# kai-neumann/OrthoSfM

Measured on AMD Instinct MI355X. Metric: image-pairs matched/sec + BA iterations/sec (N images, M tracks) at 1/2/4/8 GPU, higher is better.
Workload: dtype i8; 1 GPU; 50 orthographic images, 20000 SIFT features/img, exhaustive matching (1225 pairs, low-res gate + two-way + cross-check + lists; SURVEY 8d's unit of work: up to, not including, RANSAC-F -- the pass through RANSAC-F is `with_geometric_verification`); views=50, features_per_view=20000, pairs=1225

## Files before the change

### orthosfm_amd/csrc/match_kernels.hip

```cpp
#include <algorithm>

#include "match_kernels.h"

namespace osfm {


typedef int v4i __attribute__((ext_vector_type(4)));
typedef int v16i __attribute__((ext_vector_type(16)));


__device__ __forceinline__ int max3i(int a, int b, int c)
{
    int r;
    asm("v_max3_i32 %0, %1, %2, %3" : "=v"(r) : "v"(a), "v"(b), "v"(c));
    return r;
}
__device__ __forceinline__ int med3a(int a, int b, int c)
{
    int r;
    asm("v_med3_i32 %0, %1, %2, %3" : "=v"(r) : "v"(a), "v"(b), "v"(c));
    return r;
}

constexpr int kGroupTiles = 8;
constexpr int kPipeGroupTiles = 16;
constexpr int kPipeTileBits = 9;
constexpr int kValNone = -(1 << 28);

template <int V> struct IntC { static constexpr int value = V; };

__device__ __forceinline__ void store_colpart(int32_t *best, int32_t *second, unsigned byte_off, const ColPart &v)
{
    int32_t *const pb = reinterpret_cast<int32_t *>(reinterpret_cast<char *>(best) + byte_off);
    int32_t *const ps = reinterpret_cast<int32_t *>(reinterpret_cast<char *>(second) + byte_off);
#ifdef OSFM_COLPART_PLAIN_STORE
    *pb = v.key_best; *ps = v.key_second;
#else
    __builtin_nontemporal_store(v.key_best, pb);
    __builtin_nontemporal_store(v.key_second, ps);
#endif
}
__device__ __forceinline__ void store_colpart_sbase(int32_t *best, int32_t *second, unsigned byte_off, const ColPart &v)
{
    asm volatile("global_store_dword %0, %1, %2 nt" :: "v"(byte_off), "v"(v.key_best), "s"(best) : "memory");
    asm volatile("global_store_dword %0, %1, %2 nt" :: "v"(byte_off), "v"(v.key_second), "s"(second) : "memory");
}

template <int CH, bool MASKED, bool RAW, bool C0>
__device__ __forceinline__ void
tile_body(const MatchProblem &pd, int rb, int seg, RowPart *__restrict__ rowparts,
    ColPart *__restrict__ colparts, char *smem, const int8_t *__restrict__ zero_tile)
{
    static_assert(!C0 || RAW, "the correction-free form needs the raw row operand");
    constexpr int D = CH * 16;
    constexpr int KS = CH / 2;
    constexpr int RPB = 16 / CH;
    constexpr int TILE_BYTES = kTileCols * D;
    constexpr int CHUNKS = kTileCols * CH;
    constexpr int CPT = CHUNKS / 256;
    constexpr int BBUF_BYTES = 2 * TILE_BYTES > 16384 ? 2 * TILE_BYTES : 16384;
    constexpr int kRawShift = C0 ? kPipeTileBits : 7;
    constexpr int kCurNone = RAW ? -(1 << (30 - kRawShift)) : kKeyNone;
    static_assert(kSegCols / kTileCols <= (1 << 7), "tile index must fit the key");
    constexpr bool PIPE = C0;
    constexpr int NCHUNK = 2 * KS;
    constexpr int RPC = 16 / NCHUNK;
    constexpr int CPC = 16 / KS;

    char *bbuf = smem;
    int *corrbuf = reinterpret_cast<int *>(smem + BBUF_BYTES);
    ColPart *colbuf = reinterpret_cast<ColPart *>(smem + BBUF_BYTES + 2 * 64 * 4);
    int *rsecbuf = reinterpret_cast<int *>(smem + BBUF_BYTES + 2 * 64 * 4 + 8 * 4 * 64 * 8);

    const int n1 = pd.n1, n2 = pd.n2, n2stride = pd.n2stride;
    const int8_t *const Bbase = C0 ? pd.B_raw : pd.B;
    const int32_t *const corrBbase = pd.corrB;
    int32_t *const colbest = reinterpret_cast<int32_t *>(colparts + pd.colpart_off) + (int64_t)rb * pd.n2stride;
    int32_t *const colsecond = colbest + (int64_t)pd.nrb * pd.n2stride;
    const int tid = threadIdx.x;
    const int wave = tid >> 6, lane = tid & 63, lr = lane & 31, lh = lane >> 5;
    const int row0 = rb * kRowsPerBlock + wave * 64;
    const int gcode = wave * 2 + lh;

    const int8_t *Abase = pd.A;
    const int32_t *corrA = pd.corrA;
    int arow0 = row0;
    if (RAW) { Abase = pd.A_raw; corrA = pd.corrA_raw; }
    else if (!MASKED && rb >= pd.nrb_main) {
        Abase = pd.A_special; corrA = pd.corrA_special;
        arow0 = (rb - pd.nrb_main) * kRowsPerBlock + wave * 64;
    }
    v4i a[2][KS];
    v16i ra[2];
#pragma unroll
    for (int rf = 0; rf < 2; ++rf) {
        const int8_t *arow = Abase + (size_t)(arow0 + rf * 32 + lr) * D;
#pragma unroll
        for (int ks = 0; ks < KS; ++ks)
            a[rf][ks] = *reinterpret_cast<const v4i *>(arow + (ks * 2 + lh) * 16);
#pragma unroll
        for (int r = 0; r < 16; ++r)
            ra[rf][r] = C0 ? 0 : corrA[arow0 + rf * 32 + (r & 3) + 8 * (r >> 2) + 4 * lh];
    }
    const v16i zero16 = {0, 0, 0, 0, 0, 0, 0, 0, 0, 0, 0, 0, 0, 0, 0, 0};
    unsigned row_valid_bits = 0xffffffffu;
    if (MASKED) {
        row_valid_bits = 0;
#pragma unroll
        for (int fr = 0; fr < 32; ++fr) {
            const int row = row0 + (fr >> 4) * 32 + (fr & 3) + 8 * ((fr >> 2) & 3) + 4 * lh;
            row_valid_bits |= (row < n1 ? 1u : 0u) << fr;
        }
    }

    v16i rbest[2], rcur[2];
#pragma unroll
    for (int rf = 0; rf < 2; ++rf)
#pragma unroll
        for (int r = 0; r < 16; ++r) {
            rbest[rf][r] = kKeyNone; rcur[rf][r] = kCurNone;
            rsecbuf[(rf * 16 + r) * 256 + tid] = kKeyNone;
        }

    const int seg_cols = pd.seg_cols;
    const int col_begin = seg * seg_cols;
    const int col_lim = min(n2, col_begin + seg_cols);
    const int ntiles = (col_lim - col_begin + kTileCols - 1) / kTileCols;

    typedef __attribute__((address_space(3))) void lds_void;
    typedef const __attribute__((address_space(1))) void glb_void;
    int wave_s = __builtin_amdgcn_readfirstlane(wave);
    if (PIPE) asm volatile("" : "+s"(wave_s));
    unsigned lane4 = (unsigned)lane * 4u;
    if (PIPE) asm volatile("" : "+v"(lane4));
    unsigned lane_off[CPT];
#pragma unroll
    for (int c = 0; c < CPT; ++c) {
        const int q = (c * 4 + wave) * 64 + lane;
        const int col = q / CH;
        const int ch = (q % CH) ^ ((col / RPB) % CH);
        lane_off[c] = (unsigned)(col * D + ch * 16);
    }
    auto dma_wait = [&](bool store_behind = false) {
        if (!PIPE) return;
#ifndef OSFM_TILE_WAIT_ALL
        if (store_behind) { asm volatile("s_waitcnt vmcnt(2)" ::: "memory"); return; }
#endif
        asm volatile("s_waitcnt vmcnt(0)" ::: "memory");
    };
    auto tile_src = [&](int t) {
        const int8_t *src = Bbase + (size_t)(col_begin + t * kTileCols) * D;
        if (PIPE && t >= ntiles) src = zero_tile;
        return src;
    };
    auto stage_tile_at = [&](const int8_t *src, int t, int buf) {
#pragma unroll
        for (int c = 0; c < CPT; ++c) {
            const int q0 = (c * 4 + wave_s) * 64;
            if (PIPE) {
                static_assert(!PIPE || RAW, "the PIPE schedule must not contain compiler-managed m0 users");
                const unsigned lds_at = (unsigned)(uintptr_t)(bbuf + buf * TILE_BYTES + q0 * 16);
                asm volatile("s_mov_b32 m0, %2\n\tglobal_load_lds_dwordx4 %0, %1"
                             :: "v"(lane_off[c]), "s"(src), "s"(lds_at) : "memory");
            } else {
                __builtin_amdgcn_global_load_lds(
                    (glb_void *)(src + lane_off[c]),
                    (lds_void *)(uintptr_t)(bbuf + buf * TILE_BYTES + q0 * 16), 16, 0, 0);
            }
        }
        if (!RAW && wave_s == 0)
            __builtin_amdgcn_global_load_lds(
                (glb_void *)(corrBbase + col_begin + t * kTileCols + lane),
                (lds_void *)(uintptr_t)(corrbuf + buf * 64), 4, 0, 0);
    };
    auto stage_tile = [&](int t, int buf) { stage_tile_at(tile_src(t), t, buf); };
    const int8_t *pf_src = nullptr;

    v4i b[2][KS];
    int cb_next[2] = {0, 0};
    auto load_b = [&](int buf, int cf) {
        const int col = cf * 32 + lr;
        const int swz = (col / RPB) % CH;
#pragma unroll
        for (int ks = 0; ks < KS; ++ks)
            b[cf][ks] = *reinterpret_cast<const v4i *>(
                bbuf + buf * TILE_BYTES + col * D + (((ks * 2 + lh) ^ swz) * 16));
        if (!RAW) cb_next[cf] = corrbuf[buf * 64 + col];
    };

    int cbj[2] = {0, 0}, cjt[2] = {0, 0};
    bool col_valid[2] = {true, true};
    int g[2] = {kValNone, kValNone};

    v16i acc0[2], acc1[2];

    auto phase = [&](auto ph_c, auto cl_c, auto mg_c, auto rs_c, auto pre_c, v16i (&cur)[2], v16i (&nxt)[2], int buf_next,
                     int tile0, int tm, int tms) {
        constexpr int PH = decltype(ph_c)::value;
        constexpr bool PRE = decltype(pre_c)::value != 0;
        constexpr int CL = decltype(cl_c)::value;
        constexpr int RS = decltype(rs_c)::value;
        constexpr bool MG = decltype(mg_c)::value != 0;
        constexpr int OF = PH ^ 1;
        int sv = 0;
        ColPart cpm[4];
        if (CL >= 0) sv = rsecbuf[(OF * 16 + CL) * 256 + tid];
        if (MG) {
#pragma unroll
            for (int w = 0; w < 4; ++w) cpm[w] = colbuf[((tm & 7) * 4 + w) * 64 + lane];
        }
#pragma unroll
        for (int i = 0; i < NCHUNK; ++i) {
            const int cf = i / KS, ks = i % KS;
            if (PRE && i == 0)
                ;
            else if (ks == 0)
                nxt[cf] = __builtin_amdgcn_mfma_i32_32x32x32_i8(a[PH ^ 1][0], b[cf][0], C0 ? zero16 : ra[PH ^ 1], 0, 0, 0);
            else
                nxt[cf] = __builtin_amdgcn_mfma_i32_32x32x32_i8(a[PH ^ 1][ks], b[cf][ks], nxt[cf], 0, 0, 0);
            if (PH == 0 && i == KS - 1) load_b(buf_next, 0);
            if (PH == 1 && i == 0) {
                __builtin_amdgcn_sched_barrier(0);
                load_b(buf_next, 1);
            }

#pragma unroll
            for (int r = i * RPC; r < (i + 1) * RPC; ++r) {
                if (RAW) {
                    if (RS >= 0 && r == RS) rcur[PH][r] = max(cur[0][r], cur[1][r]);
                    else rcur[PH][r] = max(max(rcur[PH][r], cur[0][r]), cur[1][r]);
                } else {
                    int k0 = (int)(((unsigned)cur[0][r] << 8) + (unsigned)cjt[0]);
                    int k1 = (int)(((unsigned)cur[1][r] << 8) + (unsigned)cjt[1]);
                    if (MASKED) {
                        k0 = col_valid[0] ? k0 : kKeyNone;
                        k1 = col_valid[1] ? k1 : kKeyNone;
                    }
                    rcur[PH][r] = max3i(rcur[PH][r], k0, k1);
                }
            }
            {
                int x[CPC];
#pragma unroll
                for (int j = 0; j < CPC; ++j) {
                    x[j] = cur[cf][ks * CPC + j];
                    if (MASKED) x[j] = ((row_valid_bits >> (PH * 16 + ks * CPC + j)) & 1u) ? x[j] : kValNone;
                }
                int gg;
                if (PH == 0 && ks == 0) gg = max(x[0], x[1]);
                else gg = max(max(g[cf], x[0]), x[1]);
#pragma unroll
                for (int j = 2; j < CPC; j += 2) gg = max(max(gg, x[j]), x[j + 1]);
                asm volatile("" : "+v"(gg));
                g[cf] = gg;
            }
            if (CL >= 0 && i == 2) {
                const int r = CL;
                const int gk = (int)(((unsigned)rcur[OF][r] << kRawShift) | (unsigned)tile0);
                rsecbuf[(OF * 16 + r) * 256 + tid] = med3a(rbest[OF][r], sv, gk);
                int nb = max(rbest[OF][r], gk);
                if (PIPE) asm volatile("" : "+v"(nb));
                rbest[OF][r] = nb;
            }
            if (MG && (i == 2 || i == 3)) {
                if (i == 2) {
                    int k1 = cpm[0].key_best, k2 = cpm[0].key_second;
#pragma unroll
                    for (int w = 1; w < 4; ++w) {
                        k2 = max(max(min(k1, cpm[w].key_best), k2), cpm[w].key_second);
                        k1 = max(k1, cpm[w].key_best);
                    }
                    cpm[0].key_best = k1; cpm[0].key_second = k2;
                } else {
                    store_colpart_sbase(colbest + col_begin + tms * kTileCols, colsecond + col_begin + tms * kTileCols, lane4, cpm[0]);
                }
            }
            __builtin_amdgcn_sched_barrier(0);
        }
    };

    auto first_mfma = [&]() {
        acc1[0] = __builtin_amdgcn_mfma_i32_32x32x32_i8(a[1][0], b[0][0], C0 ? zero16 : ra[1], 0, 0, 0);
        __builtin_amdgcn_sched_barrier(0);
    };

    stage_tile(0, 0);
    stage_tile(PIPE || ntiles > 1 ? 1 : 0, 1);
    dma_wait();
    __syncthreads();
    load_b(0, 0);
    load_b(0, 1);
#pragma unroll
    for (int cf = 0; cf < 2; ++cf) {
        acc0[cf] = __builtin_amdgcn_mfma_i32_32x32x32_i8(a[0][0], b[cf][0], C0 ? zero16 : ra[0], 0, 0, 0);
#pragma unroll
        for (int ks = 1; ks < KS; ++ks)
            acc0[cf] = __builtin_amdgcn_mfma_i32_32x32x32_i8(a[0][ks], b[cf][ks], acc0[cf], 0, 0, 0);
    }
    if (PIPE) {
        first_mfma();
        pf_src = tile_src(2);
        asm volatile("" : "+s"(pf_src));
    }
    __syncthreads();

    auto tile_top = [&](int t) {
        if (PIPE) {
            stage_tile_at(pf_src, t + 2, t & 1);
            pf_src = tile_src(t + 3);
            asm volatile("" : "+s"(pf_src));
        } else {
            stage_tile(min(t + 2, ntiles - 1), t & 1);
        }
#pragma unroll
        for (int cf = 0; cf < 2; ++cf) {
            if (!RAW) {
                cbj[cf] = cb_next[cf];
                cjt[cf] = (int)(((unsigned)cbj[cf] << 8) + (unsigned)(t * 2 + cf));
                asm volatile("" : "+v"(cjt[cf]));
            }
            col_valid[cf] = (col_begin + t * kTileCols + cf * 32 + lr) < n2;
        }
    };
    auto tile_bottom = [&](int t, bool store_behind = false, bool pre_issue = false) {
        int kk[2];
#pragma unroll
        for (int cf = 0; cf < 2; ++cf) {
            kk[cf] = (int)((unsigned)(g[cf] + cbj[cf]) << 8) | gcode;
            if (MASKED) kk[cf] = g[cf] < -(1 << 27) ? kKeyNone : kk[cf];
        }
        const auto sw = __builtin_amdgcn_permlane32_swap((unsigned)kk[0], (unsigned)kk[1], false, false);
        const int x0 = (int)sw[0], x1 = (int)sw[1];
        ColPart cp;
        cp.key_best = max(x0, x1);
        cp.key_second = min(x0, x1);
        colbuf[((t & 7) * 4 + wave) * 64 + lane] = cp;
        if (pre_issue) first_mfma();
        dma_wait(store_behind);
        __syncthreads();
    };
    auto close_all = [&](auto first_tile) {
        int sv[2][16];
#pragma unroll
        for (int rf = 0; rf < 2; ++rf)
#pragma unroll
            for (int r = 0; r < 16; ++r) sv[rf][r] = rsecbuf[(rf * 16 + r) * 256 + tid];
#pragma unroll
        for (int rf = 0; rf < 2; ++rf)
#pragma unroll
            for (int r = 0; r < 16; ++r) {
                const int gk = RAW ? (int)(((unsigned)rcur[rf][r] << kRawShift) | (unsigned)first_tile(rf, r)) : rcur[rf][r];
                rsecbuf[(rf * 16 + r) * 256 + tid] = med3a(rbest[rf][r], sv[rf][r], gk);
                rbest[rf][r] = max(rbest[rf][r], gk);
                rcur[rf][r] = kCurNone;
            }
    };
    auto merge_tile = [&](int tm) {
        ColPart cp[4];
#pragma unroll
        for (int w = 0; w < 4; ++w) cp[w] = colbuf[((tm & 7) * 4 + w) * 64 + lane];
        int k1 = cp[0].key_best, k2 = cp[0].key_second;
#pragma unroll
        for (int w = 1; w < 4; ++w) {
            k2 = max(max(min(k1, cp[w].key_best), k2), cp[w].key_second);
            k1 = max(k1, cp[w].key_best);
        }
        const int col = col_begin + tm * kTileCols + lane;
        if (col < n2stride) {
            ColPart out;
            out.key_best = k1;
            out.key_second = k2;
            store_colpart(colbest, colsecond, (unsigned)col * 4u, out);
        }
    };

    int t = 0;
    if (PIPE) {
        static_assert(kPipeGroupTiles == 16, "the staggered schedule closes one of 16 slots per phase");
        auto cycle_tile = [&](auto u_c, int t0) {
            constexpr int u = decltype(u_c)::value;
            const int tt = t0 + u;
            tile_top(tt);
            const int bn = (tt & 1) ^ 1;
            const int tm0 = u >= 5 ? tt - 5 : max(tt - 5, 0);
            const int tm = tm0 + wave;
            phase(IntC<0>(), IntC<u>(), IntC<(u & 3) == 1 ? 1 : 0>(), IntC<(u + 15) & 15>(), IntC<1>(), acc0, acc1, bn,
                max(tt - 16, 0), tm, tm0 + wave_s);
            phase(IntC<1>(), IntC<u>(), IntC<0>(), IntC<u>(), IntC<0>(), acc1, acc0, bn, max(tt - 15, 0), 0, 0);
            tile_bottom(tt, (u & 3) == 1, true);
            return tt + 1 >= ntiles;
        };
        for (; t + 16 < ntiles; t += 16) {
            cycle_tile(IntC<0>(), t); cycle_tile(IntC<1>(), t); cycle_tile(IntC<2>(), t); cycle_tile(IntC<3>(), t);
            cycle_tile(IntC<4>(), t); cycle_tile(IntC<5>(), t); cycle_tile(IntC<6>(), t); cycle_tile(IntC<7>(), t);
            cycle_tile(IntC<8>(), t); cycle_tile(IntC<9>(), t); cycle_tile(IntC<10>(), t); cycle_tile(IntC<11>(), t);
            cycle_tile(IntC<12>(), t); cycle_tile(IntC<13>(), t); cycle_tile(IntC<14>(), t); cycle_tile(IntC<15>(), t);
        }
        do {
            if (cycle_tile(IntC<0>(), t)) break;
            if (cycle_tile(IntC<1>(), t)) break;
            if (cycle_tile(IntC<2>(), t)) break;
            if (cycle_tile(IntC<3>(), t)) break;
            if (cycle_tile(IntC<4>(), t)) break;
            if (cycle_tile(IntC<5>(), t)) break;
            if (cycle_tile(IntC<6>(), t)) break;
            if (cycle_tile(IntC<7>(), t)) break;
            if (cycle_tile(IntC<8>(), t)) break;
            if (cycle_tile(IntC<9>(), t)) break;
            if (cycle_tile(IntC<10>(), t)) break;
            if (cycle_tile(IntC<11>(), t)) break;
            if (cycle_tile(IntC<12>(), t)) break;
            if (cycle_tile(IntC<13>(), t)) break;
            if (cycle_tile(IntC<14>(), t)) break;
            cycle_tile(IntC<15>(), t);
        } while (false);
        const int tl = ntiles - 1, ue = tl & 15, t0 = tl & ~15;
        const int tf = max((tl - 1) & ~3, 0);
        if (tf + wave_s <= tl) merge_tile(tf + wave_s);
        if (tf + 4 + wave_s <= tl) merge_tile(tf + 4 + wave_s);
#pragma unroll
        for (int r = 0; r < 16; ++r) rcur[0][r] = r == ue ? kCurNone : rcur[0][r];
        close_all([&](int rf, int r) {
            if (rf) return r <= ue ? t0 + r : max(t0 - 16 + r, 0);
            return r < ue ? t0 + r + 1 : r > ue ? max(t0 - 15 + r, 0) : 0;
        });
        t = ntiles;
        dma_wait();
    }
    const int t_tail = t;
    if (!PIPE)
    for (; t < ntiles; ++t) {
        tile_top(t);
        phase(IntC<0>(), IntC<-1>(), IntC<0>(), IntC<-1>(), IntC<0>(), acc0, acc1, (t & 1) ^ 1, 0, 0, 0);
        phase(IntC<1>(), IntC<-1>(), IntC<0>(), IntC<-1>(), IntC<0>(), acc1, acc0, (t & 1) ^ 1, 0, 0, 0);
        if (PIPE ? t == ntiles - 1 : ((t % kGroupTiles) == kGroupTiles - 1 || t == ntiles - 1)) {
            const int first = PIPE ? t_tail : (t / kGroupTiles) * kGroupTiles;
            close_all([&](int, int) { return first; });
        }
        tile_bottom(t);
        if ((t & 3) == 3 || t == ntiles - 1) {
            const int tm = (t & ~3) + wave;
            if (tm <= t) merge_tile(tm);
        }
    }

    RowPart *rp = rowparts + pd.rowpart_off + (int64_t)seg * ((int64_t)pd.nrb * kRowsPerBlock);
    int *bb = reinterpret_cast<int *>(smem);
    static_assert(BBUF_BYTES + 2 * 64 * 4 + 8 * 4 * 64 * 8 >= 32 * 256 * 4, "the best keys of both fragments must fit in front of rsecbuf");
    __syncthreads();
#pragma unroll
    for (int rf = 0; rf < 2; ++rf)
#pragma unroll
        for (int r = 0; r < 16; ++r) bb[(rf * 16 + r) * 256 + tid] = rbest[rf][r];
    __syncthreads();
    {
        constexpr int SH = RAW ? kRawShift : 8;
        const int r = lane & 15, h = (lane >> 4) & 1, rf = lane >> 5;
        const int base = (rf * 16 + r) * 256 + wave * 64 + h * 32;
        v4i kb[8], ks[8];
#pragma unroll
        for (int j = 0; j < 8; ++j) {
            const int jj = (j + r) & 7;
            kb[j] = *reinterpret_cast<const v4i *>(bb + base + jj * 4);
            ks[j] = *reinterpret_cast<const v4i *>(rsecbuf + base + jj * 4);
        }
        int b1 = kKeyNone, b2 = kKeyNone, smax = kKeyNone;
#pragma unroll
        for (int j = 0; j < 8; ++j)
#pragma unroll
            for (int e = 0; e < 4; ++e) {
                b2 = med3a(b1, b2, kb[j][e]);
                b1 = max(b1, kb[j][e]);
            }
#pragma unroll
        for (int j = 0; j < 8; j += 2)
#pragma unroll
            for (int e = 0; e < 4; ++e) smax = max3i(smax, ks[j][e], ks[j + 1][e]);
        unsigned hit = 0;
#pragma unroll
        for (int j = 7; j >= 0; --j)
#pragma unroll
            for (int e = 3; e >= 0; --e) hit = (hit << 1) | (kb[j][e] == b1 ? 1u : 0u);
        const unsigned rot = __builtin_amdgcn_alignbit(hit, hit, (32 - 4 * r) & 31);
        const int bl = 31 - __builtin_clz(rot | 1u);
        const int sk = max(b2, smax);
        const int row = row0 + rf * 32 + (r & 3) + 8 * (r >> 2) + 4 * h;
        RowPart out;
        out.ip_best = b1 == kKeyNone ? INT_MIN : (b1 >> SH);
        out.ip_second = sk == kKeyNone ? INT_MIN : (sk >> SH);
        out.idx_best = b1 == kKeyNone ? 0
                     : RAW ? col_begin + (b1 & ((1 << kRawShift) - 1)) * kTileCols + bl
                           : col_begin + (b1 & 255) * 32 + bl;
        out.pad = RAW ? 1 : 0;
        rp[row] = out;
    }
}

template <int CH, bool MASKED, bool RAW, bool C0>
__global__ __launch_bounds__(256, 2) void
match_tile_kernel(const MatchProblem *__restrict__ problems, int num_problems, int total_blocks,
    RowPart *__restrict__ rowparts, ColPart *__restrict__ colparts, unsigned long long *__restrict__ clock_probe,
    const int8_t *__restrict__ zero_tile)
{
    extern __shared__ __attribute__((aligned(16))) char smem[];
    const int lin = xcd_remap(blockIdx.x, total_blocks);
    int lo = 0, hi = num_problems - 1;
    while (lo < hi) {
        const int mid = (lo + hi + 1) >> 1;
        if (problems[mid].block_start <= lin) lo = mid; else hi = mid - 1;
    }
    const MatchProblem &pd = problems[lo];
    const int local = lin - pd.block_start;
    const int rb = local / pd.nseg;
    const int seg = local - rb * pd.nseg;
    if (!MASKED && (rb < pd.nrb_main) != RAW) return;
    if (RAW && (pd.c0 != 0) != C0) return;
    if (C0 && clock_probe != nullptr && (blockIdx.x & 1023) == 0) {
        const unsigned long long c0 = (unsigned long long)clock64(), w0 = (unsigned long long)wall_clock64();
        tile_body<CH, MASKED, RAW, C0>(pd, rb, seg, rowparts, colparts, smem, zero_tile);
        const unsigned long long c1 = (unsigned long long)clock64(), w1 = (unsigned long long)wall_clock64();
        if (threadIdx.x == 0) { atomicAdd(clock_probe, c1 - c0); atomicAdd(clock_probe + 1, w1 - w0); }
        return;
    }
    tile_body<CH, MASKED, RAW, C0>(pd, rb, seg, rowparts, colparts, smem, zero_tile);
}

void launch_match_tiles(int ch, bool masked, bool any_special, bool any_c0, bool any_corrected,
    const MatchProblem *d_problems, int num_problems, int total_blocks, RowPart *rowparts,
    ColPart *colparts, hipStream_t s, unsigned long long *clock_probe, const int8_t *zero_tile)
{
    if (total_blocks <= 0) return;
    const int d = ch * 16;
    const size_t lds = std::max<size_t>(2 * (size_t)kTileCols * d, 16384) + 2 * 64 * 4 + 8 * 4 * 64 * sizeof(ColPart) + 32 * 256 * 4;
    const dim3 grid(total_blocks), block(256);
#define OSFM_LAUNCH_TILES(CHV, MASKEDV, RAWV, C0V) \
    for (unsigned long long *PROBE = ((C0V) ? clock_probe : nullptr), *once_ = (unsigned long long *)1; once_; once_ = nullptr) \
    hipLaunchKernelGGL((match_tile_kernel<CHV, MASKEDV, RAWV, C0V>), grid, block, lds, s, d_problems, num_problems, total_blocks, rowparts, colparts, PROBE, zero_tile)
    if (masked) {
        if (ch == 8) OSFM_LAUNCH_TILES(8, true, false, false); else OSFM_LAUNCH_TILES(4, true, false, false);
        return;
    }
    if (any_c0) { if (ch == 8) OSFM_LAUNCH_TILES(8, false, true, true); else OSFM_LAUNCH_TILES(4, false, true, true); }
    if (any_corrected) { if (ch == 8) OSFM_LAUNCH_TILES(8, false, true, false); else OSFM_LAUNCH_TILES(4, false, true, false); }
    if (any_special) { if (ch == 8) OSFM_LAUNCH_TILES(8, false, false, false); else OSFM_LAUNCH_TILES(4, false, false, false); }
#undef OSFM_LAUNCH_TILES
}

__device__ __forceinline__ int match_distance(int ip, const LoweTable &tab)
{
    const int b = max(ip, 0);
    return tab.is_signed ? 32258 - 2 * min(b, 16129) : min(32767, 65025 - min(b, 65025)) * 2;
}

__device__ __forceinline__ int
accept_match(int ip1, int ip2, int idx1, const LoweTable &tab)
{
    const int idx = ip1 >= 0 ? idx1 : 0;
    const int d1 = match_distance(ip1, tab), d2 = match_distance(ip2, tab);
    if (d1 > tab.max_d1) return -1;
    if (d1 >= tab.reject_from[d2 >> 1]) return -1;
    return idx;
}

template <int CTRL, int ROW_MASK = 0xf>
__device__ __forceinline__ int dpp_mov(int v, int old)
{
    return __builtin_amdgcn_update_dpp(old, v, CTRL, ROW_MASK, 0xf, false);
}
constexpr int kDppXor1 = 0xB1;
constexpr int kDppXor2 = 0x4E;
constexpr int kDppHalfMirror = 0x141;
constexpr int kDppMirror = 0x140;
constexpr int kDppBcast15 = 0x142;
constexpr int kDppBcast31 = 0x143;

__device__ __forceinline__ int wave_max(int v)
{
    v = max(v, dpp_mov<kDppXor1>(v, INT_MIN));
    v = max(v, dpp_mov<kDppXor2>(v, INT_MIN));
    v = max(v, dpp_mov<kDppHalfMirror>(v, INT_MIN));
    v = max(v, dpp_mov<kDppMirror>(v, INT_MIN));
    v = max(v, dpp_mov<kDppBcast15, 0xa>(v, INT_MIN));
    v = max(v, dpp_mov<kDppBcast31, 0xc>(v, INT_MIN));
    return __builtin_amdgcn_readlane(v, 63);
}

template <int DIM, int DIR>
__device__ __forceinline__ void
rescan_groups(const MatchProblem &pd, const int (&q)[2], const int (&idx1)[2], const int (&code)[2],
    const int (&kind)[2], int lane, int (&idx_out)[2], int (&best_out)[2], int (&second_out)[2])
{
    constexpr int LPC = DIM / 16;
    constexpr int CPL = 64 / LPC;
    constexpr int NCAND = DIR == 0 ? 2 * kPipeGroupTiles : 32;
    constexpr int J = NCAND / CPL;
    const int c = lane % LPC, k = lane / LPC;
    const int8_t *Q = DIR == 0 ? pd.A : pd.B;
    const int8_t *Cm = DIR == 0 ? pd.B : pd.A;
    const int32_t *corrQ = DIR == 0 ? pd.corrA : pd.corrB;
    const int32_t *corrC = DIR == 0 ? pd.corrB : pd.corrA;

    int cand[2][J], corr_c[2][J], corr_q[2];
    int4 qv[2], cv[2][J];
#pragma unroll
    for (int u = 0; u < 2; ++u) {
        qv[u] = *reinterpret_cast<const int4 *>(Q + (size_t)q[u] * DIM + c * 16);
        corr_q[u] = corrQ[q[u]];
        int base0 = 0, lr = 0, rbase = 0, lh = 0;
        if (DIR == 0) {
            const int seg = idx1[u] / kSegCols, off = idx1[u] - seg * kSegCols;
            lr = off & 31;
            const int tile = off >> 6;
            base0 = seg * kSegCols + (kind[u] ? tile : (tile / kGroupTiles) * kGroupTiles) * kTileCols;
        } else {
            rbase = idx1[u] * kRowsPerBlock + (code[u] >> 1) * 64;
            lh = code[u] & 1;
        }
#pragma unroll
        for (int j = 0; j < J; ++j) {
            const int n = j * CPL + k;
            int cd;
            if (kind[u] >= 3) {
                cd = idx1[u] + (kind[u] == 3 ? 128 : 32) * n;
                if (cd >= (DIR == 0 ? pd.n2 : pd.n1)) cd = -1;
            } else if (DIR == 0) {
                cd = base0 + (n >> 1) * kTileCols + (n & 1) * 32 + lr;
                if (cd >= pd.n2 || (!kind[u] && n >= 2 * kGroupTiles)) cd = -1;
            } else {
                const int r = n & 15;
                cd = rbase + (n >> 4) * 32 + (r & 3) + 8 * (r >> 2) + 4 * lh;
                if (idx1[u] < pd.nrb_main && cd >= pd.n1) cd = -1;
            }
            cand[u][j] = cd;
        }
        if (DIR == 1 && kind[u] < 3 && idx1[u] >= pd.nrb_main) {
#pragma unroll
            for (int j = 0; j < J; ++j) {
                const int sidx = cand[u][j] - pd.nrb_main * kRowsPerBlock;
                cand[u][j] = sidx < pd.n_special ? pd.special_map[sidx] : -1;
            }
        }
    }
#pragma unroll
    for (int u = 0; u < 2; ++u) {
#pragma unroll
        for (int j = 0; j < J; ++j) {
            const int cs = max(cand[u][j], 0);
            cv[u][j] = *reinterpret_cast<const int4 *>(Cm + (size_t)cs * DIM + c * 16);
            corr_c[u][j] = corrC[cs];
        }
    }
#pragma unroll
    for (int u = 0; u < 2; ++u) {
        int kbest = INT_MIN, ksec = INT_MIN;
#pragma unroll
        for (int j = 0; j < J; ++j) {
            int acc = __builtin_amdgcn_sdot4(qv[u].x, cv[u][j].x, 0, false);
            acc = __builtin_amdgcn_sdot4(qv[u].y, cv[u][j].y, acc, false);
            acc = __builtin_amdgcn_sdot4(qv[u].z, cv[u][j].z, acc, false);
            acc = __builtin_amdgcn_sdot4(qv[u].w, cv[u][j].w, acc, false);
            acc += dpp_mov<kDppXor1>(acc, 0);
            acc += dpp_mov<kDppXor2>(acc, 0);
            if (LPC == 8) acc += dpp_mov<kDppHalfMirror>(acc, 0);
            const int key = cand[u][j] >= 0 ? (acc + corr_q[u] + corr_c[u][j]) * 32 + (j * CPL + k) : INT_MIN;
            ksec = med3a(kbest, ksec, key);
            kbest = max(kbest, key);
        }
        const int wbest = wave_max(kbest);
        const int wsec = wave_max(kbest == wbest ? ksec : kbest);
        const int pos = wbest & 31;
        int widx = 0;
#pragma unroll
        for (int j = 0; j < J; ++j)
            if ((pos / CPL) == j) widx = __builtin_amdgcn_readlane(cand[u][j], (pos % CPL) * LPC);
        idx_out[u] = max(widx, 0);
        best_out[u] = wbest >> 5;
        second_out[u] = wsec == INT_MIN ? INT_MIN : wsec >> 5;
    }
}

template <int DIM>
__device__ __forceinline__ void
scan_specials(const MatchProblem &pd, int dir, int q, int lane, int &best_out, int &second_out, int &idx_out)
{
    constexpr int LPC = DIM / 16, CPL = 64 / LPC;
    const int c = lane % LPC, k = lane / LPC;
    const int8_t *Q = dir == 0 ? pd.A : pd.B;
    const int8_t *Cm = dir == 0 ? pd.B_special : pd.A_special;
    const int32_t *corrC = dir == 0 ? pd.corrB_special : pd.corrA_special;
    const int32_t *map = dir == 0 ? pd.special_map_B : pd.special_map;
    const int ns = dir == 0 ? pd.nsB : pd.nsA;
    const int4 qv = *reinterpret_cast<const int4 *>(Q + (size_t)q * DIM + c * 16);
    const int corr_q = (dir == 0 ? pd.corrA : pd.corrB)[q];
    int kbest = INT_MIN, ksec = INT_MIN;
    for (int base = 0; base < ns; base += CPL) {
        const int slot = base + k;
        const bool live = slot < ns;
        const int4 cv = *reinterpret_cast<const int4 *>(Cm + (size_t)(live ? slot : 0) * DIM + c * 16);
        int acc = __builtin_amdgcn_sdot4(qv.x, cv.x, 0, false);
        acc = __builtin_amdgcn_sdot4(qv.y, cv.y, acc, false);
        acc = __builtin_amdgcn_sdot4(qv.z, cv.z, acc, false);
        acc = __builtin_amdgcn_sdot4(qv.w, cv.w, acc, false);
        acc += dpp_mov<kDppXor1>(acc, 0);
        acc += dpp_mov<kDppXor2>(acc, 0);
        if (LPC == 8) acc += dpp_mov<kDppHalfMirror>(acc, 0);
        const int key = live ? (acc + corr_q + corrC[live ? slot : 0]) * 512 + slot : INT_MIN;
        ksec = med3a(kbest, ksec, key);
        kbest = max(kbest, key);
    }
    const int wbest = wave_max(kbest);
    const int wsec = wave_max(kbest == wbest ? ksec : kbest);
    best_out = wbest >> 9;
    second_out = wsec == INT_MIN ? INT_MIN : wsec >> 9;
    idx_out = map[wbest & 511];
}

#ifndef OSFM_FINISH_BATCH
#define OSFM_FINISH_BATCH 16
#endif

constexpr int kFinishThreads = 256, kFinishTurns = 4, kFinishSpan = kFinishThreads * kFinishTurns;

template <int DIM, bool SIGNED>
__global__ __launch_bounds__(kFinishThreads) void
match_finish_kernel(const MatchProblem *__restrict__ problems, const RowPart *__restrict__ rowparts,
    const ColPart *__restrict__ colparts, const RowPart *__restrict__ sp_parts, const int32_t *__restrict__ sp_col,
    LoweTable tab, int force_exact, ExactItem *__restrict__ exact_items, int32_t *__restrict__ exact_count, int exact_cap,
    int32_t *__restrict__ rs_count, RescoreItem *__restrict__ rs_items, int spans_per_dir, int total_blocks)
{
    const int lin = xcd_remap(blockIdx.x, total_blocks);
    const int problem = lin / (2 * spans_per_dir), within = lin - problem * 2 * spans_per_dir;
    const MatchProblem &pd = problems[problem];
    const int dir = within / spans_per_dir;
    const int span = within - dir * spans_per_dir;
    const int lane = threadIdx.x & 63;
    const int nq = dir == 0 ? pd.n1 : pd.n2;
    const int nc = dir == 0 ? pd.n2 : pd.n1;
    int32_t *out = dir == 0 ? pd.m12 : pd.m21;
    const int limit = tab.is_signed ? 32767 : 65535;
#pragma unroll 1
    for (int q0 = span * kFinishSpan; q0 < min(nq, (span + 1) * kFinishSpan); q0 += kFinishThreads) {
        const int q = q0 + (int)threadIdx.x;
        const bool active = q < nq;

        int ip1 = INT_MIN, ip2 = INT_MIN, idx1 = 0, code = 0, kind1 = 0;
        int sp_slot = -1;
        if (active && nc > 0 && pd.sp) {
            const int ns_mine = dir == 0 ? pd.nsA : pd.nsB;
            if (ns_mine > 0) sp_slot = (dir == 0 ? pd.special_slot : pd.special_slot_B)[q];
            if (sp_slot >= 0) {
                const int ns_pad = (ns_mine + 31) & ~31;
                const int chunk_cols = pd.sp_wide[dir] ? kSpWideChunk : kSpChunk;
                const int nchunk = (nc + chunk_cols - 1) / chunk_cols;
                const RowPart *rp0 = sp_parts + pd.sp_row_off[dir] + sp_slot;
                for (int c = 0; c < nchunk; ++c) {
                    const RowPart p = rp0[(int64_t)c * ns_pad];
                    ip2 = max(max(ip2, p.ip_second), min(ip1, p.ip_best));
                    if (p.ip_best >= ip1 && p.ip_best != INT_MIN) { ip1 = p.ip_best; idx1 = p.idx_best; }
                }
                kind1 = pd.sp_wide[dir] ? 4 : 3;
            }
        }
        bool sp_scan = false;
        bool failed = false;
        int sp_m1 = INT_MIN;
        if (active && nc > 0 && sp_slot < 0) {
            if (dir == 0) {
                const int64_t stride = (int64_t)pd.nrb * kRowsPerBlock;
                int slot = q;
                if (pd.special_slot && !pd.sp) {
                    const int sidx = pd.special_slot[q];
                    if (sidx >= 0) slot = pd.nrb_main * kRowsPerBlock + sidx;
                }
                constexpr int kBatch = 4;
                const RowPart *rp0 = rowparts + pd.rowpart_off + slot;
                const int nseg = pd.nseg;
                for (int s0 = 0; s0 < nseg; s0 += kBatch) {
                    RowPart p[kBatch];
#pragma unroll
                    for (int u = 0; u < kBatch; ++u) p[u] = rp0[(int64_t)min(s0 + u, nseg - 1) * stride];
                    __builtin_amdgcn_sched_barrier(0);
#pragma unroll
                    for (int u = 0; u < kBatch; ++u) {
                        const bool live = s0 + u < nseg;
                        const int pb = live ? p[u].ip_best : INT_MIN, ps = live ? p[u].ip_second : INT_MIN;
                        ip2 = max(max(ip2, ps), min(ip1, pb));
                        if (pb >= ip1 && pb != INT_MIN) { ip1 = pb; idx1 = p[u].idx_best; kind1 = p[u].pad; }
                    }
                }
            } else {
                constexpr int kBatch = OSFM_FINISH_BATCH;
                const int32_t *best0 = reinterpret_cast<const int32_t *>(colparts + pd.colpart_off) + q;
                const int nrb = pd.nrb;
                const int64_t stride = pd.n2stride;
                for (int rb0 = 0; rb0 < nrb; rb0 += kBatch) {
                    int kb[kBatch];
#pragma unroll
                    for (int u = 0; u < kBatch; ++u)
                        kb[u] = __builtin_nontemporal_load(best0 + (int64_t)min(rb0 + u, nrb - 1) * stride);
                    __builtin_amdgcn_sched_barrier(0);
#pragma unroll
                    for (int u = 0; u < kBatch; ++u) {
                        const bool live = rb0 + u < nrb;
                        const int pb = (!live || kb[u] == kKeyNone) ? INT_MIN : (kb[u] >> 8);
                        ip2 = max(ip2, min(ip1, pb));
                        if (pb >= ip1 && pb != INT_MIN) { ip1 = pb; idx1 = rb0 + u; code = kb[u] & 255; }
                    }
                }
                if (!(force_exact || pd.force_exact || ip1 > limit || (pd.sp && pd.nsA > 0))) {
                    const int d1 = match_distance(ip1, tab);
                    failed = d1 > tab.max_d1 || d1 >= tab.reject_from[match_distance(ip2, tab) >> 1];
                }
                if (ip1 != INT_MIN && !failed) {
                    const int ks = __builtin_nontemporal_load(best0 + ((int64_t)nrb + idx1) * stride);
                    ip2 = max(ip2, ks == kKeyNone ? INT_MIN : (ks >> 8));
                }
            }
            if (pd.sp && (dir == 0 ? pd.nsB : pd.nsA) > 0) {
                const int t1 = sp_col[pd.sp_col_off[dir ^ 1] + q];
                if (t1 >= ip1 && t1 != INT_MIN) {
                    sp_m1 = ip1; ip1 = t1; sp_scan = true;
                } else {
                    ip2 = max(ip2, t1);
                }
            }
        }
        bool exact = active && nc > 0 && (force_exact || pd.force_exact || ip1 > limit);
        bool refine = false;
        int res = -1;
        if (active && nc > 0 && !exact) {
            res = failed ? -1 : accept_match(ip1, sp_scan ? max(sp_m1, ip2) : ip2, 0, tab);
            if (res >= 0) {
                if (ip1 < 0) { res = 0; sp_scan = false; }
                else if ((sp_scan ? sp_m1 : ip2) == ip1) { exact = true; sp_scan = false; }
                else if (!sp_scan) refine = true;
            } else {
                sp_scan = false;
            }
        } else {
            sp_scan = false;
// ... 688 lines not shown
```

Measured before the change: 24790 pairs/s.

## Spread next-tile DMA pieces across MFMA chunks in pipelined tile loop

Splits the per-tile global-to-LDS prefetch into two pieces issued at chosen MFMA chunk positions inside phase 0, instead of issuing both at the top of each tile. The vmcnt wait count becomes a compile-time value that accounts for the column-part stores still in flight. This spreads memory issue across the compute schedule to reduce stalls at the tile top. It also adds an optional timestamp instrumentation path compiled only under a debug macro. Moving the prefetch later shortens the time the load has to land before the end-of-tile wait, which could expose latency.

```diff
diff --git a/orthosfm_amd/csrc/match_kernels.hip b/orthosfm_amd/csrc/match_kernels.hip
--- a/orthosfm_amd/csrc/match_kernels.hip
+++ b/orthosfm_amd/csrc/match_kernels.hip
@@ -28,6 +28,19 @@
 constexpr int kValNone = -(1 << 28);
 
 template <int V> struct IntC { static constexpr int value = V; };
+
+constexpr int kDmaPieceAt[2] = {1, 2};
+static_assert(kDmaPieceAt[0] >= -1 && kDmaPieceAt[0] <= kDmaPieceAt[1] && kDmaPieceAt[1] < 16, "piece 0 is issued first");
+constexpr int kColStoreAt = 3;
+
+#ifdef OSFM_TILE_STAMPS
+constexpr bool kTileStamps = true;
+#else
+constexpr bool kTileStamps = false;
+#endif
+constexpr int kStampsPerTile = 10;
+enum { kStTileStart = 0, kStPiece0Pre, kStPiece0Post, kStPiece1Pre, kStPiece1Post, kStPhase0End, kStPhase1End,
+       kStWaitPre, kStWaitPost, kStBarrierPost };
 
 __device__ __forceinline__ void store_colpart(int32_t *best, int32_t *second, unsigned byte_off, const ColPart &v)
 {
@@ -46,10 +59,10 @@
     asm volatile("global_store_dword %0, %1, %2 nt" :: "v"(byte_off), "v"(v.key_second), "s"(second) : "memory");
 }
 
-template <int CH, bool MASKED, bool RAW, bool C0>
+template <int CH, bool MASKED, bool RAW, bool C0, bool ST = false>
 __device__ __forceinline__ void
 tile_body(const MatchProblem &pd, int rb, int seg, RowPart *__restrict__ rowparts,
-    ColPart *__restrict__ colparts, char *smem, const int8_t *__restrict__ zero_tile)
+    ColPart *__restrict__ colparts, char *smem, const int8_t *__restrict__ zero_tile, unsigned *wg_stamps = nullptr)
 {
     static_assert(!C0 || RAW, "the correction-free form needs the raw row operand");
     constexpr int D = CH * 16;
@@ -141,21 +154,22 @@
         const int ch = (q % CH) ^ ((col / RPB) % CH);
         lane_off[c] = (unsigned)(col * D + ch * 16);
     }
-    auto dma_wait = [&](bool store_behind = false) {
+    auto dma_wait = [&](auto younger_c) {
         if (!PIPE) return;
 #ifndef OSFM_TILE_WAIT_ALL
-        if (store_behind) { asm volatile("s_waitcnt vmcnt(2)" ::: "memory"); return; }
+        constexpr int N = decltype(younger_c)::value;
+#else
+        constexpr int N = 0;
 #endif
-        asm volatile("s_waitcnt vmcnt(0)" ::: "memory");
+        asm volatile("s_waitcnt vmcnt(%0)" :: "n"(N) : "memory");
     };
     auto tile_src = [&](int t) {
         const int8_t *src = Bbase + (size_t)(col_begin + t * kTileCols) * D;
         if (PIPE && t >= ntiles) src = zero_tile;
         return src;
     };
-    auto stage_tile_at = [&](const int8_t *src, int t, int buf) {
-#pragma unroll
-        for (int c = 0; c < CPT; ++c) {
+    auto stage_piece = [&](int c, const int8_t *src, int buf) {
+        {
             const int q0 = (c * 4 + wave_s) * 64;
             if (PIPE) {
                 static_assert(!PIPE || RAW, "the PIPE schedule must not contain compiler-managed m0 users");
@@ -168,6 +182,10 @@
                     (lds_void *)(uintptr_t)(bbuf + buf * TILE_BYTES + q0 * 16), 16, 0, 0);
             }
         }
+    };
+    auto stage_tile_at = [&](const int8_t *src, int t, int buf) {
+#pragma unroll
+        for (int c = 0; c < CPT; ++c) stage_piece(c, src, buf);
         if (!RAW && wave_s == 0)
             __builtin_amdgcn_global_load_lds(
                 (glb_void *)(corrBbase + col_begin + t * kTileCols + lane),
@@ -175,6 +193,28 @@
     };
     auto stage_tile = [&](int t, int buf) { stage_tile_at(tile_src(t), t, buf); };
     const int8_t *pf_src = nullptr;
+    constexpr bool PLACED = PIPE && CPT == 2;
+    constexpr int P0_AT = PLACED ? kDmaPieceAt[0] : -1, P1_AT = PLACED ? kDmaPieceAt[1] : -1;
+    constexpr int STORES_BEHIND = kColStoreAt > P1_AT ? 2 : 0;
+    constexpr bool STAMPED = kTileStamps && PLACED && ST;
+    constexpr int STAMPS_BEHIND = 3 + (P1_AT < NCHUNK ? 1 : 0);
+#ifdef OSFM_TILE_STAMPS
+    unsigned *const stamp_slot = wg_stamps + wave_s * (16 * kStampsPerTile);
+    unsigned *stamp_base = stamp_slot;
+#endif
+    auto stamp = [&](auto on_c, auto slot_c) {
+#ifdef OSFM_TILE_STAMPS
+        if constexpr (decltype(on_c)::value != 0) {
+            unsigned long long tk;
+            __builtin_amdgcn_sched_barrier(0);
+            asm volatile("s_memtime %0\n\ts_waitcnt lgkmcnt(0)" : "=s"(tk) :: "memory");
+            const unsigned lo = (unsigned)tk;
+            asm volatile("s_mov_b64 exec, 1\n\tglobal_store_dword %0, %1, %2 offset:%3\n\ts_mov_b64 exec, -1"
+                         :: "v"(lane4), "v"(lo), "s"(stamp_base), "n"(decltype(slot_c)::value * 4) : "memory");
+            __builtin_amdgcn_sched_barrier(0);
+        }
+#endif
+    };
 
     v4i b[2][KS];
     int cb_next[2] = {0, 0};
@@ -194,7 +234,7 @@
 
     v16i acc0[2], acc1[2];
 
-    auto phase = [&](auto ph_c, auto cl_c, auto mg_c, auto rs_c, auto pre_c, v16i (&cur)[2], v16i (&nxt)[2], int buf_next,
+    auto phase = [&](auto ph_c, auto cl_c, auto mg_c, auto rs_c, auto pre_c, auto st_c, v16i (&cur)[2], v16i (&nxt)[2], int buf_next,
                      int tile0, int tm, int tms) {
         constexpr int PH = decltype(ph_c)::value;
         constexpr bool PRE = decltype(pre_c)::value != 0;
@@ -275,8 +315,22 @@
                     store_colpart_sbase(colbest + col_begin + tms * kTileCols, colsecond + col_begin + tms * kTileCols, lane4, cpm[0]);
                 }
             }
+            if constexpr (PLACED && CL >= 0) {
+                constexpr int S0 = (CL >= 0 ? CL : 0) * kStampsPerTile;
+                if (P0_AT == PH * NCHUNK + i) {
+                    stamp(st_c, IntC<S0 + kStPiece0Pre>());
+                    stage_piece(0, pf_src, buf_next ^ 1);
+                    if (P1_AT != P0_AT) stamp(st_c, IntC<S0 + kStPiece0Post>());
+                }
+                if (P1_AT == PH * NCHUNK + i) {
+                    if (P1_AT != P0_AT) stamp(st_c, IntC<S0 + kStPiece1Pre>());
+                    stage_piece(1, pf_src, buf_next ^ 1);
+                    stamp(st_c, IntC<S0 + kStPiece1Post>());
+                }
+            }
             __builtin_amdgcn_sched_barrier(0);
         }
+        if constexpr (CL >= 0) stamp(st_c, IntC<(CL >= 0 ? CL : 0) * kStampsPerTile + (PH ? kStPhase1End : kStPhase0End)>());
     };
 
     auto first_mfma = [&]() {
@@ -286,7 +340,7 @@
 
     stage_tile(0, 0);
     stage_tile(PIPE || ntiles > 1 ? 1 : 0, 1);
-    dma_wait();
+    dma_wait(IntC<0>());
     __syncthreads();
     load_b(0, 0);
     load_b(0, 1);
@@ -304,11 +358,25 @@
     }
     __syncthreads();
 
-    auto tile_top = [&](int t) {
+    auto next_src = [&](int t) {
+        pf_src = tile_src(t + 3);
+        asm volatile("" : "+s"(pf_src));
+    };
+    auto tile_top = [&](int t, auto st_c, auto u_c) {
         if (PIPE) {
-            stage_tile_at(pf_src, t + 2, t & 1);
-            pf_src = tile_src(t + 3);
-            asm volatile("" : "+s"(pf_src));
+            constexpr int S0 = decltype(u_c)::value * kStampsPerTile;
+            stamp(st_c, IntC<S0 + kStTileStart>());
+            if (P0_AT < 0) {
+                stamp(st_c, IntC<S0 + kStPiece0Pre>());
+                if (PLACED) stage_piece(0, pf_src, t & 1);
+                else stage_tile_at(pf_src, t + 2, t & 1);
+                if (P1_AT >= 0) stamp(st_c, IntC<S0 + kStPiece0Post>());
+            }
+            if (PLACED && P1_AT < 0) {
+                stage_piece(1, pf_src, t & 1);
+                stamp(st_c, IntC<S0 + kStPiece1Post>());
+            }
+            if (P1_AT < 0) next_src(t);
         } else {
             stage_tile(min(t + 2, ntiles - 1), t & 1);
         }
@@ -322,7 +390,8 @@
             col_valid[cf] = (col_begin + t * kTileCols + cf * 32 + lr) < n2;
         }
     };
-    auto tile_bottom = [&](int t, bool store_behind = false, bool pre_issue = false) {
+    auto tile_bottom = [&](int t, auto younger_c, auto st_c, auto u_c, bool pre_issue = false) {
+        constexpr int S0 = decltype(u_c)::value * kStampsPerTile;
         int kk[2];
 #pragma unroll
         for (int cf = 0; cf < 2; ++cf) {
@@ -336,8 +405,11 @@
         cp.key_second = min(x0, x1);
         colbuf[((t & 7) * 4 + wave) * 64 + lane] = cp;
         if (pre_issue) first_mfma();
-        dma_wait(store_behind);
+        stamp(st_c, IntC<S0 + kStWaitPre>());
+        dma_wait(younger_c);
+        stamp(st_c, IntC<S0 + kStWaitPost>());
         __syncthreads();
+        stamp(st_c, IntC<S0 + kStBarrierPost>());
     };
     auto close_all = [&](auto first_tile) {
         int sv[2][16];
@@ -377,42 +449,60 @@
     int t = 0;
     if (PIPE) {
         static_assert(kPipeGroupTiles == 16, "the staggered schedule closes one of 16 slots per phase");
-        auto cycle_tile = [&](auto u_c, int t0) {
+        auto cycle_tile = [&](auto u_c, int t0, auto st_c) {
             constexpr int u = decltype(u_c)::value;
+            constexpr bool MGT = (u & 3) == 1;
+            constexpr int YOUNGER = (MGT ? STORES_BEHIND : 0) + (decltype(st_c)::value ? STAMPS_BEHIND : 0);
             const int tt = t0 + u;
-            tile_top(tt);
+            tile_top(tt, st_c, u_c);
             const int bn = (tt & 1) ^ 1;
             const int tm0 = u >= 5 ? tt - 5 : max(tt - 5, 0);
             const int tm = tm0 + wave;
-            phase(IntC<0>(), IntC<u>(), IntC<(u & 3) == 1 ? 1 : 0>(), IntC<(u + 15) & 15>(), IntC<1>(), acc0, acc1, bn,
+            phase(IntC<0>(), IntC<u>(), IntC<MGT ? 1 : 0>(), IntC<(u + 15) & 15>(), IntC<1>(), st_c, acc0, acc1, bn,
                 max(tt - 16, 0), tm, tm0 + wave_s);
-            phase(IntC<1>(), IntC<u>(), IntC<0>(), IntC<u>(), IntC<0>(), acc1, acc0, bn, max(tt - 15, 0), 0, 0);
-            tile_bottom(tt, (u & 3) == 1, true);
+            if (P1_AT >= 0 && P1_AT < NCHUNK) next_src(tt);
+            phase(IntC<1>(), IntC<u>(), IntC<0>(), IntC<u>(), IntC<0>(), st_c, acc1, acc0, bn, max(tt - 15, 0), 0, 0);
+            if (P1_AT >= NCHUNK) next_src(tt);
+            tile_bottom(tt, IntC<YOUNGER>(), st_c, u_c, true);
             return tt + 1 >= ntiles;
         };
+        constexpr IntC<0> NS{};
+        auto whole_cycle = [&](auto st_c) {
+            cycle_tile(IntC<0>(), t, st_c); cycle_tile(IntC<1>(), t, st_c); cycle_tile(IntC<2>(), t, st_c); cycle_tile(IntC<3>(), t, st_c);
+            cycle_tile(IntC<4>(), t, st_c); cycle_tile(IntC<5>(), t, st_c); cycle_tile(IntC<6>(), t, st_c); cycle_tile(IntC<7>(), t, st_c);
+            cycle_tile(IntC<8>(), t, st_c); cycle_tile(IntC<9>(), t, st_c); cycle_tile(IntC<10>(), t, st_c); cycle_tile(IntC<11>(), t, st_c);
+            cycle_tile(IntC<12>(), t, st_c); cycle_tile(IntC<13>(), t, st_c); cycle_tile(IntC<14>(), t, st_c); cycle_tile(IntC<15>(), t, st_c);
+        };
+#ifdef OSFM_TILE_STAMPS
+        const int nfree = (ntiles - 1) / 16;
+        const int t_stamp = nfree >= 2 ? 16 * (nfree / 2) : -1;
+#endif
         for (; t + 16 < ntiles; t += 16) {
-            cycle_tile(IntC<0>(), t); cycle_tile(IntC<1>(), t); cycle_tile(IntC<2>(), t); cycle_tile(IntC<3>(), t);
-            cycle_tile(IntC<4>(), t); cycle_tile(IntC<5>(), t); cycle_tile(IntC<6>(), t); cycle_tile(IntC<7>(), t);
-            cycle_tile(IntC<8>(), t); cycle_tile(IntC<9>(), t); cycle_tile(IntC<10>(), t); cycle_tile(IntC<11>(), t);
-            cycle_tile(IntC<12>(), t); cycle_tile(IntC<13>(), t); cycle_tile(IntC<14>(), t); cycle_tile(IntC<15>(), t);
+#ifdef OSFM_TILE_STAMPS
+            if constexpr (STAMPED) {
+                stamp_base = stamp_slot + (t == t_stamp ? 0 : 4 * 16 * kStampsPerTile);
+                asm volatile("" : "+s"(stamp_base));
+            }
+#endif
+            whole_cycle(IntC<STAMPED ? 1 : 0>());
         }
         do {
-            if (cycle_tile(IntC<0>(), t)) break;
-            if (cycle_tile(IntC<1>(), t)) break;
-            if (cycle_tile(IntC<2>(), t)) break;
-            if (cycle_tile(IntC<3>(), t)) break;
-            if (cycle_tile(IntC<4>(), t)) break;
-            if (cycle_tile(IntC<5>(), t)) break;
-            if (cycle_tile(IntC<6>(), t)) break;
-            if (cycle_tile(IntC<7>(), t)) break;
-            if (cycle_tile(IntC<8>(), t)) break;
-            if (cycle_tile(IntC<9>(), t)) break;
-            if (cycle_tile(IntC<10>(), t)) break;
-            if (cycle_tile(IntC<11>(), t)) break;
-            if (cycle_tile(IntC<12>(), t)) break;
-            if (cycle_tile(IntC<13>(), t)) break;
-            if (cycle_tile(IntC<14>(), t)) break;
-            cycle_tile(IntC<15>(), t);
+            if (cycle_tile(IntC<0>(), t, NS)) break;
+            if (cycle_tile(IntC<1>(), t, NS)) break;
+            if (cycle_tile(IntC<2>(), t, NS)) break;
+            if (cycle_tile(IntC<3>(), t, NS)) break;
+            if (cycle_tile(IntC<4>(), t, NS)) break;
+            if (cycle_tile(IntC<5>(), t, NS)) break;
+            if (cycle_tile(IntC<6>(), t, NS)) break;
+            if (cycle_tile(IntC<7>(), t, NS)) break;
+            if (cycle_tile(IntC<8>(), t, NS)) break;
+            if (cycle_tile(IntC<9>(), t, NS)) break;
+            if (cycle_tile(IntC<10>(), t, NS)) break;
+            if (cycle_tile(IntC<11>(), t, NS)) break;
+            if (cycle_tile(IntC<12>(), t, NS)) break;
+            if (cycle_tile(IntC<13>(), t, NS)) break;
+            if (cycle_tile(IntC<14>(), t, NS)) break;
+            cycle_tile(IntC<15>(), t, NS);
         } while (false);
         const int tl = ntiles - 1, ue = tl & 15, t0 = tl & ~15;
         const int tf = max((tl - 1) & ~3, 0);
@@ -425,19 +515,19 @@
             return r < ue ? t0 + r + 1 : r > ue ? max(t0 - 15 + r, 0) : 0;
         });
         t = ntiles;
-        dma_wait();
+        dma_wait(IntC<0>());
     }
     const int t_tail = t;
     if (!PIPE)
     for (; t < ntiles; ++t) {
-        tile_top(t);
-        phase(IntC<0>(), IntC<-1>(), IntC<0>(), IntC<-1>(), IntC<0>(), acc0, acc1, (t & 1) ^ 1, 0, 0, 0);
-        phase(IntC<1>(), IntC<-1>(), IntC<0>(), IntC<-1>(), IntC<0>(), acc1, acc0, (t & 1) ^ 1, 0, 0, 0);
+        tile_top(t, IntC<0>(), IntC<0>());
+        phase(IntC<0>(), IntC<-1>(), IntC<0>(), IntC<-1>(), IntC<0>(), IntC<0>(), acc0, acc1, (t & 1) ^ 1, 0, 0, 0);
+        phase(IntC<1>(), IntC<-1>(), IntC<0>(), IntC<-1>(), IntC<0>(), IntC<0>(), acc1, acc0, (t & 1) ^ 1, 0, 0, 0);
         if (PIPE ? t == ntiles - 1 : ((t % kGroupTiles) == kGroupTiles - 1 || t == ntiles - 1)) {
             const int first = PIPE ? t_tail : (t / kGroupTiles) * kGroupTiles;
             close_all([&](int, int) { return first; });
         }
-        tile_bottom(t);
+        tile_bottom(t, IntC<0>(), IntC<0>(), IntC<0>());
         if ((t & 3) == 3 || t == ntiles - 1) {
             const int tm = (t & ~3) + wave;
             if (tm <= t) merge_tile(tm);
@@ -500,7 +590,11 @@
 __global__ __launch_bounds__(256, 2) void
 match_tile_kernel(const MatchProblem *__restrict__ problems, int num_problems, int total_blocks,
     RowPart *__restrict__ rowparts, ColPart *__restrict__ colparts, unsigned long long *__restrict__ clock_probe,
-    const int8_t *__restrict__ zero_tile)
+    const int8_t *__restrict__ zero_tile
+#ifdef OSFM_TILE_STAMPS
+    , unsigned *tile_stamps, int stamp_slots
+#endif
+    )
 {
     extern __shared__ __attribute__((aligned(16))) char smem[];
     const int lin = xcd_remap(blockIdx.x, total_blocks);
@@ -515,6 +609,13 @@
     const int seg = local - rb * pd.nseg;
     if (!MASKED && (rb < pd.nrb_main) != RAW) return;
     if (RAW && (pd.c0 != 0) != C0) return;
+#ifdef OSFM_TILE_STAMPS
+    if (C0 && tile_stamps != nullptr && (blockIdx.x & 1023) == 0 && (int)(blockIdx.x >> 10) < stamp_slots) {
+        tile_body<CH, MASKED, RAW, C0, true>(pd, rb, seg, rowparts, colparts, smem, zero_tile,
+            tile_stamps + (size_t)(blockIdx.x >> 10) * (2 * 4 * 16 * kStampsPerTile));
+        return;
+    }
+#endif
     if (C0 && clock_probe != nullptr && (blockIdx.x & 1023) == 0) {
         const unsigned long long c0 = (unsigned long long)clock64(), w0 = (unsigned long long)wall_clock64();
         tile_body<CH, MASKED, RAW, C0>(pd, rb, seg, rowparts, colparts, smem, zero_tile);
@@ -525,6 +626,27 @@
     tile_body<CH, MASKED, RAW, C0>(pd, rb, seg, rowparts, colparts, smem, zero_tile);
 }
 
+#ifdef OSFM_TILE_STAMPS
+static unsigned *g_tile_stamps = nullptr;
+static int g_tile_stamp_slots = 0, g_tile_stamp_launches = 0, g_tile_stamp_launch = 0;
+extern "C" __attribute__((visibility("default"))) int osfm_debug_set_tile_stamps(void *device_buffer, int slots_per_launch, int launches)
+{
+    g_tile_stamps = static_cast<unsigned *>(device_buffer);
+    g_tile_stamp_slots = device_buffer ? slots_per_launch : 0;
+    g_tile_stamp_launches = device_buffer ? launches : 0;
+    g_tile_stamp_launch = 0;
+    return kStampsPerTile;
+}
+static unsigned *next_tile_stamps(bool c0)
+{
+    if (!c0 || g_tile_stamps == nullptr || g_tile_stamp_launch >= g_tile_stamp_launches) return nullptr;
+    return g_tile_stamps + (size_t)(g_tile_stamp_launch++) * g_tile_stamp_slots * (2 * 4 * 16 * kStampsPerTile);
+}
+#define OSFM_STAMP_ARGS(C0V) , next_tile_stamps(C0V), g_tile_stamp_slots
+#else
+#define OSFM_STAMP_ARGS(C0V)
+#endif
+
 void launch_match_tiles(int ch, bool masked, bool any_special, bool any_c0, bool any_corrected,
     const MatchProblem *d_problems, int num_problems, int total_blocks, RowPart *rowparts,
     ColPart *colparts, hipStream_t s, unsigned long long *clock_probe, const int8_t *zero_tile)
@@ -535,7 +657,7 @@
     const dim3 grid(total_blocks), block(256);
 #define OSFM_LAUNCH_TILES(CHV, MASKEDV, RAWV, C0V) \
     for (unsigned long long *PROBE = ((C0V) ? clock_probe : nullptr), *once_ = (unsigned long long *)1; once_; once_ = nullptr) \
-    hipLaunchKernelGGL((match_tile_kernel<CHV, MASKEDV, RAWV, C0V>), grid, block, lds, s, d_problems, num_problems, total_blocks, rowparts, colparts, PROBE, zero_tile)
+    hipLaunchKernelGGL((match_tile_kernel<CHV, MASKEDV, RAWV, C0V>), grid, block, lds, s, d_problems, num_problems, total_blocks, rowparts, colparts, PROBE, zero_tile OSFM_STAMP_ARGS(C0V))
     if (masked) {
         if (ch == 8) OSFM_LAUNCH_TILES(8, true, false, false); else OSFM_LAUNCH_TILES(4, true, false, false);
         return;
```

After: 25030 pairs/s (median of 6 runs). No clear change (+1.0%).
